# Tom-Ryder/VIforSDEs

Measured on AMD Instinct MI355X. Metric: sampled-paths/sec + ELBO-iters/sec (value = global_batch * ELBO-iters/s), higher is better.
Workload: dtype f32 (GRU/ELBO kernels) + bf16-autocast encoder; 1 GPU; lv: state_dim=2, T=400 (dt=0.1), batch=512/GPU, enc 256x8x4 heads, GRU 64x2; global_batch=512, parallelism=dp1, hip_graph=True

## Files before the change

### viforsdes_amd/csrc/vsde_common.h

```cpp
#pragma once
#include <hip/hip_runtime.h>
#include <stdint.h>
#include <stdio.h>
#include <stdlib.h>

#include "../../include/vsde_hip.h"

namespace vsde {

constexpr int kWave = 64;
constexpr int kHP = 64;
constexpr int kChunks = 16;
constexpr int kMatF4 = kChunks * 3 * kHP;

void set_error(const char *fmt, ...);

#ifdef VSDE_ABLATIONS
static inline long long vsde_knob(const char *name, long long dflt) {
    const char *e = getenv(name);
    return (e && *e) ? atoll(e) : dflt;
}
static inline int ablation_env(const char *name) {
    const char *e = getenv(name);
    const int v = e ? atoi(e) : 0;
// ... 22 lines not shown
        }                                                                            \
    } while (0)

struct RowView {
    const void *base;
    int64_t batch_stride;
    int64_t row_stride;
    int rows_per_batch;
    int shift;
    int col_split;
    int col_skip;
    int dtype;
};

__device__ __forceinline__ float bf16_to_f32(uint16_t v) { return __uint_as_float(((uint32_t)v) << 16); }

__device__ __forceinline__ int64_t rowview_offset(const RowView &v, int m, bool &valid) {
    int b = m / v.rows_per_batch;
    int t = m - b * v.rows_per_batch + v.shift;
    valid = t >= 0;
    return (int64_t)b * v.batch_stride + (int64_t)t * v.row_stride;
}

__device__ __forceinline__ float rowview_load(const RowView &v, int64_t off, int k) {
    int kk = k < v.col_split ? k : k + v.col_skip;
    if (v.dtype == 0) return ((const float *)v.base)[off + kk];
    return bf16_to_f32(((const uint16_t *)v.base)[off + kk]);
}

__device__ __forceinline__ float fast_rcp(float x) { return __builtin_amdgcn_rcpf(x); }
// ... 121 lines not shown
```

### viforsdes_amd/csrc/vsde_encoder.hip

```cpp
#include <stdlib.h>

#include "vsde_common.h"

namespace vsde {

struct bf16_t { uint16_t v; };

__device__ __forceinline__ float to_f32(float x) { return x; }
__device__ __forceinline__ float to_f32(bf16_t x) { return __uint_as_float(((uint32_t)x.v) << 16); }
template <typename T> __device__ __forceinline__ T from_f32(float x);
template <> __device__ __forceinline__ float from_f32<float>(float x) { return x; }
template <> __device__ __forceinline__ bf16_t from_f32<bf16_t>(float x) {
    uint32_t u = __float_as_uint(x);
    if ((u & 0x7fffffffu) > 0x7f800000u) return bf16_t{(uint16_t)((u >> 16) | 0x40)};
    u += 0x7fffu + ((u >> 16) & 1u);
    return bf16_t{(uint16_t)(u >> 16)};
}
template <typename T> __device__ __forceinline__ float rnd(float x) { return to_f32(from_f32<T>(x)); }

__device__ __forceinline__ float sigm(float x) { return fast_rcp(1.0f + __expf(-x)); }

template <typename T, int V> struct Pack;
template <int V> struct Pack<float, V> {
    static __device__ __forceinline__ void load(const float *p, float (&o)[V]) {
        if (V == 4) { float4 t = *(const float4 *)p; o[0] = t.x; o[1] = t.y; o[2] = t.z; o[3] = t.w; }
        else if (V == 2) { float2 t = *(const float2 *)p; o[0] = t.x; o[1] = t.y; }
        else {
#pragma unroll
            for (int i = 0; i < V; ++i) o[i] = p[i];
        }
    }
    static __device__ __forceinline__ void store(float *p, const float (&o)[V]) {
        if (V == 4) *(float4 *)p = make_float4(o[0], o[1], o[2], o[3]);
        else if (V == 2) *(float2 *)p = make_float2(o[0], o[1]);
        else {
#pragma unroll
            for (int i = 0; i < V; ++i) p[i] = o[i];
        }
    }
};
template <int V> struct Pack<bf16_t, V> {
    static __device__ __forceinline__ void load(const bf16_t *p, float (&o)[V]) {
        if (V == 8) { uint4 t = *(const uint4 *)p; const uint32_t w[4] = {t.x, t.y, t.z, t.w};
#pragma unroll
            for (int i = 0; i < 4; ++i) { o[2 * i] = __uint_as_float(w[i] << 16); o[2 * i + 1] = __uint_as_float(w[i] & 0xffff0000u); } }
        else if (V == 4) { uint2 t = *(const uint2 *)p; const uint32_t w[2] = {t.x, t.y};
#pragma unroll
            for (int i = 0; i < 2; ++i) { o[2 * i] = __uint_as_float(w[i] << 16); o[2 * i + 1] = __uint_as_float(w[i] & 0xffff0000u); } }
        else if (V == 2) { uint32_t w = *(const uint32_t *)p; o[0] = __uint_as_float(w << 16); o[1] = __uint_as_float(w & 0xffff0000u); }
        else {
#pragma unroll
            for (int i = 0; i < V; ++i) o[i] = to_f32(p[i]);
        }
    }
    static __device__ __forceinline__ void store(bf16_t *p, const float (&o)[V]) {
        if (V == 8 || V == 4 || V == 2) {
            uint32_t w[V / 2 > 0 ? V / 2 : 1];
#pragma unroll
            for (int i = 0; i < V / 2; ++i) w[i] = (uint32_t)from_f32<bf16_t>(o[2 * i]).v | ((uint32_t)from_f32<bf16_t>(o[2 * i + 1]).v << 16);
            if (V == 8) *(uint4 *)p = make_uint4(w[0], w[1], w[2 % (V / 2)], w[3 % (V / 2)]);
            else if (V == 4) *(uint2 *)p = make_uint2(w[0], w[1 % (V / 2)]);
            else *(uint32_t *)p = w[0];
        } else {
#pragma unroll
            for (int i = 0; i < V; ++i) p[i] = from_f32<bf16_t>(o[i]);
        }
    }
};
template <typename T> struct VecOf { static constexpr int v = 4; };
template <> struct VecOf<bf16_t> { static constexpr int v = 8; };

__device__ __forceinline__ float seg_sum(float v, int width) {
    for (int off = width >> 1; off > 0; off >>= 1) v += __shfl_xor(v, off, 64);
    return v;
}

template <typename T, int V, int LPR, int NSLAB>
__global__ void __launch_bounds__(256) ln_mod_fwd_kernel(const T *__restrict__ x, const T *__restrict__ scale,
                                                         const T *__restrict__ shift, T *__restrict__ y,
                                                         float *__restrict__ mean, float *__restrict__ rstd, int64_t M,
                                                         int N, int C, float eps, const T *__restrict__ res_y,
                                                         const T *__restrict__ res_gate, T *__restrict__ xnew, int64_t mp) {
    const int lane = threadIdx.x & (LPR - 1);
    constexpr int nslab = NSLAB;
    const int64_t stride = (int64_t)gridDim.x * (256 / LPR);
    int64_t m = (int64_t)blockIdx.x * (256 / LPR) + threadIdx.x / LPR;
    float v[NSLAB][V], ry[NSLAB][V], nv[NSLAB][V], nry[NSLAB][V];
    auto fetch = [&](int64_t mm, float (&vx)[NSLAB][V], float (&vy)[NSLAB][V]) {
#pragma unroll
        for (int sl = 0; sl < NSLAB; ++sl)
            if (sl < nslab) {
                Pack<T, V>::load(x + mm * C + (sl * LPR + lane) * V, vx[sl]);
                if (res_y) Pack<T, V>::load(res_y + mm * C + (sl * LPR + lane) * V, vy[sl]);
            }
    };
    if (m < M) fetch(m, v, ry);
    for (; m < M; m += stride) {
        const int64_t mn = m + stride;
        if (mn < M) fetch(mn, nv, nry);
        const int64_t b = m / N;
        float s = 0.f;
#pragma unroll
        for (int sl = 0; sl < NSLAB; ++sl)
            if (sl < nslab) {
                if (res_y) {
                    float rg[V];
                    Pack<T, V>::load(res_gate + b * mp + (sl * LPR + lane) * V, rg);
#pragma unroll
                    for (int e = 0; e < V; ++e) v[sl][e] = rnd<T>(v[sl][e] + rnd<T>(rg[e] * ry[sl][e]));
                    Pack<T, V>::store(xnew + m * C + (sl * LPR + lane) * V, v[sl]);
                }
#pragma unroll
                for (int e = 0; e < V; ++e) s += v[sl][e];
            }
        const float mu = seg_sum(s, LPR) / C;
        float q = 0.f;
#pragma unroll
        for (int sl = 0; sl < NSLAB; ++sl)
            if (sl < nslab)
#pragma unroll
                for (int e = 0; e < V; ++e) { const float d = v[sl][e] - mu; q += d * d; }
        const float rs = rsqrtf(seg_sum(q, LPR) / C + eps);
        if (lane == 0) { mean[m] = mu; rstd[m] = rs; }
#pragma unroll
        for (int sl = 0; sl < NSLAB; ++sl)
            if (sl < nslab) {
                const int c = (sl * LPR + lane) * V;
                float sc[V], sh[V], o[V];
                Pack<T, V>::load(scale + b * mp + c, sc); Pack<T, V>::load(shift + b * mp + c, sh);
#pragma unroll
                for (int e = 0; e < V; ++e) o[e] = (v[sl][e] - mu) * rs * (1.0f + sc[e]) + sh[e];
                Pack<T, V>::store(y + m * C + c, o);
            }
#pragma unroll
        for (int sl = 0; sl < NSLAB; ++sl)
#pragma unroll
            for (int e = 0; e < V; ++e) { v[sl][e] = nv[sl][e]; ry[sl][e] = nry[sl][e]; }
    }
}

constexpr int kColsumChunksMax = 64;
static int colsum_chunks(int64_t B, int N) {
    static int force = -1;
    if (force < 0) force = (int)vsde_knob("VSDE_COLSUM_CHUNKS", 0);
    if (force > 0) return force > kColsumChunksMax ? kColsumChunksMax : (force > N ? (N > 0 ? N : 1) : force);
    int64_t c = (768 + B - 1) / B;
    if (c < 4) c = 4;
    if (c > kColsumChunksMax) c = kColsumChunksMax;
    if (c > N / 8) c = N / 8 > 0 ? N / 8 : 1;
    return (int)c;
}

template <int NACC>
__device__ __forceinline__ void colsum_block_reduce(float *red, const float (&acc)[NACC], int slot, int slots, int lane_off,
                                                    int width, float *__restrict__ part, int C) {
    __syncthreads();
#pragma unroll
    for (int e = 0; e < NACC; ++e) red[slot * width + lane_off + e] = acc[e];
    __syncthreads();
    for (int c = threadIdx.x; c < width && c < C; c += blockDim.x) {
        float t = 0.f;
        for (int sidx = 0; sidx < slots; ++sidx) t += red[sidx * width + c];
        part[c] = t;
    }
}

template <typename T, int V, int LPR, int NSLAB>
__global__ void __launch_bounds__(256) ln_mod_bwd_kernel(const T *__restrict__ x, const T *__restrict__ scale,
                                                         const T *__restrict__ dy, const float *__restrict__ mean,
                                                         const float *__restrict__ rstd, const T *__restrict__ dres,
                                                         T *__restrict__ dx, float *__restrict__ part, int N, int C,
                                                         const T *__restrict__ res_y, const T *__restrict__ res_gate,
                                                         T *__restrict__ res_dy, int64_t mp) {
    extern __shared__ float red[];
    constexpr int SLOTS = 256 / LPR;
    const int lane = threadIdx.x & (LPR - 1), slot = threadIdx.x / LPR;
    const int b = blockIdx.y, nchunk = gridDim.x, B = gridDim.y;
    const int CL = (N + nchunk - 1) / nchunk;
    const int n0 = blockIdx.x * CL, n1 = min(N, n0 + CL);
    constexpr int nslab = NSLAB;
    float sc1[NSLAB][V], a1[NSLAB][V], a2[NSLAB][V], a3[NSLAB][V], gt[NSLAB][V];
#pragma unroll
    for (int sl = 0; sl < NSLAB; ++sl) {
        if (sl < nslab) {
            Pack<T, V>::load(scale + (int64_t)b * mp + (sl * LPR + lane) * V, sc1[sl]);
#pragma unroll
            for (int e = 0; e < V; ++e) sc1[sl][e] += 1.0f;
            if (res_y) Pack<T, V>::load(res_gate + (int64_t)b * mp + (sl * LPR + lane) * V, gt[sl]);
        }
#pragma unroll
        for (int e = 0; e < V; ++e) { a1[sl][e] = 0.f; a2[sl][e] = 0.f; a3[sl][e] = 0.f; }
    }
    for (int n = n0 + slot; n < n1; n += SLOTS) {
        const int64_t m = (int64_t)b * N + n;
        const float mu = mean[m], rs = rstd[m];
        float g[NSLAB][V], xh[NSLAB][V];
        float s1 = 0.f, s2 = 0.f;
#pragma unroll
        for (int sl = 0; sl < NSLAB; ++sl)
            if (sl < nslab) {
                const int c = (sl * LPR + lane) * V;
                Pack<T, V>::load(x + m * C + c, xh[sl]); Pack<T, V>::load(dy + m * C + c, g[sl]);
#pragma unroll
                for (int e = 0; e < V; ++e) {
                    xh[sl][e] = (xh[sl][e] - mu) * rs;
                    a1[sl][e] += g[sl][e] * xh[sl][e]; a2[sl][e] += g[sl][e];
                    g[sl][e] *= sc1[sl][e];
                    s1 += g[sl][e]; s2 += g[sl][e] * xh[sl][e];
                }
            }
        s1 = seg_sum(s1, LPR) / C; s2 = seg_sum(s2, LPR) / C;
#pragma unroll
        for (int sl = 0; sl < NSLAB; ++sl)
            if (sl < nslab) {
                const int c = (sl * LPR + lane) * V;
                float o[V];
#pragma unroll
                for (int e = 0; e < V; ++e) o[e] = rs * (g[sl][e] - s1 - xh[sl][e] * s2);
                if (dres) {
                    float r[V];
                    Pack<T, V>::load(dres + m * C + c, r);
#pragma unroll
                    for (int e = 0; e < V; ++e) o[e] += r[e];
                }
                Pack<T, V>::store(dx + m * C + c, o);
                if (res_y) {
                    float ry[V], od[V];
                    Pack<T, V>::load(res_y + m * C + c, ry);
#pragma unroll
                    for (int e = 0; e < V; ++e) { const float t = rnd<T>(o[e]); a3[sl][e] += t * ry[e]; od[e] = gt[sl][e] * t; }
                    Pack<T, V>::store(res_dy + m * C + c, od);
                }
            }
    }
    float *p0 = part + (((int64_t)0 * B + b) * nchunk + blockIdx.x) * C;
    float *p1 = part + (((int64_t)1 * B + b) * nchunk + blockIdx.x) * C;
#pragma unroll
    for (int sl = 0; sl < NSLAB; ++sl)
        if (sl < nslab) {
            const int off = sl * LPR * V;
            colsum_block_reduce<V>(red, a1[sl], slot, SLOTS, lane * V, LPR * V, p0 + off, C - off);
            colsum_block_reduce<V>(red, a2[sl], slot, SLOTS, lane * V, LPR * V, p1 + off, C - off);
            if (res_y) {
                float *p2 = part + (((int64_t)2 * B + b) * nchunk + blockIdx.x) * C;
                colsum_block_reduce<V>(red, a3[sl], slot, SLOTS, lane * V, LPR * V, p2 + off, C - off);
            }
        }
}

template <typename T, int V>
__global__ void __launch_bounds__(256) gated_residual_bwd_kernel(const T *__restrict__ y, const T *__restrict__ gate,
                                                                 const T *__restrict__ dout, T *__restrict__ dy,
                                                                 float *__restrict__ part, int N, int C, int64_t mp) {
    extern __shared__ float red[];
    const int lpt = C / V;
    const int slots = 256 / lpt;
    const int slot = threadIdx.x / lpt, lane = threadIdx.x - slot * lpt;
    const int b = blockIdx.y, nchunk = gridDim.x;
    const int CL = (N + nchunk - 1) / nchunk;
    const int n0 = blockIdx.x * CL, n1 = min(N, n0 + CL);
    const bool live = slot < slots;
    float gv[V], acc[V];
// ... 48 lines not shown
}

template <typename T, int V>
__global__ void __launch_bounds__(256) gated_residual_kernel(const T *__restrict__ x, const T *__restrict__ y,
                                                             const T *__restrict__ gate, T *__restrict__ out, int64_t total,
                                                             int N, int C, int mode, int64_t mp) {
    const int64_t stride = (int64_t)gridDim.x * blockDim.x * V;
    for (int64_t i0 = ((int64_t)blockIdx.x * blockDim.x + threadIdx.x) * V; i0 < total; i0 += stride) {
        const int64_t m = i0 / C;
        const int c = (int)(i0 - m * C);
        const int64_t b = m / N;
        float gv[V], yv[V], xv[V], o[V];
        Pack<T, V>::load(gate + b * mp + c, gv); Pack<T, V>::load(y + i0, yv);
        if (mode == 0) Pack<T, V>::load(x + i0, xv);
#pragma unroll
        for (int e = 0; e < V; ++e) { const float g = gv[e] * yv[e]; o[e] = mode == 0 ? xv[e] + rnd<T>(g) : g; }
        Pack<T, V>::store(out + i0, o);
    }
}

template <typename T, int V>
__global__ void __launch_bounds__(256) swiglu_fwd_kernel(const T *__restrict__ u, T *__restrict__ out, int64_t M, int H2) {
    const int hv = H2 / V;
    const int64_t total = M * hv, stride = (int64_t)gridDim.x * blockDim.x;
    for (int64_t i = (int64_t)blockIdx.x * blockDim.x + threadIdx.x; i < total; i += stride) {
        const int64_t m = i / hv;
        const int j = (int)(i - m * hv) * V;
        float a[V], bv[V], o[V];
        Pack<T, V>::load(u + m * 2 * H2 + j, a); Pack<T, V>::load(u + m * 2 * H2 + H2 + j, bv);
#pragma unroll
        for (int e = 0; e < V; ++e) o[e] = rnd<T>(a[e] * sigm(a[e])) * bv[e];
        Pack<T, V>::store(out + m * H2 + j, o);
    }
}

template <typename T, int V>
__global__ void __launch_bounds__(256) swiglu_bwd_kernel(const T *__restrict__ u, const T *__restrict__ dout, T *__restrict__ du,
                                                         int64_t M, int H2) {
    const int hv = H2 / V;
    const int64_t total = M * hv, stride = (int64_t)gridDim.x * blockDim.x;
    for (int64_t i = (int64_t)blockIdx.x * blockDim.x + threadIdx.x; i < total; i += stride) {
        const int64_t m = i / hv;
        const int j = (int)(i - m * hv) * V;
        float a[V], bv[V], g[V], da[V], db[V];
        Pack<T, V>::load(u + m * 2 * H2 + j, a); Pack<T, V>::load(u + m * 2 * H2 + H2 + j, bv); Pack<T, V>::load(dout + m * H2 + j, g);
#pragma unroll
// ... 7 lines not shown

template <typename T, int V>
__global__ void __launch_bounds__(256) gate_merge_fwd_kernel(const T *__restrict__ attn, const T *__restrict__ glog,
                                                             T *__restrict__ out, int64_t M, int N, int heads, int d, int token_major,
                                                             int64_t gstride) {
    const int C = heads * d, cv = C / V;
    const int64_t total = M * cv, stride = (int64_t)gridDim.x * blockDim.x;
    for (int64_t i = (int64_t)blockIdx.x * blockDim.x + threadIdx.x; i < total; i += stride) {
        const int64_t m = i / cv;
        const int c = (int)(i - m * cv) * V, hh = c / d, k = c - hh * d;
        const int64_t b = m / N, n = m - b * N;
        float gl[V], av[V], o[V];
        Pack<T, V>::load(glog + m * gstride + k, gl);
        Pack<T, V>::load(attn + (token_major ? m * C + c : ((b * heads + hh) * N + n) * d + k), av);
#pragma unroll
        for (int e = 0; e < V; ++e) o[e] = av[e] * rnd<T>(sigm(gl[e]));
        Pack<T, V>::store(out + m * C + c, o);
    }
}

template <typename T, int V>
__global__ void __launch_bounds__(256) gate_merge_bwd_kernel(const T *__restrict__ attn, const T *__restrict__ glog,
                                                             const T *__restrict__ dout, T *__restrict__ dattn,
                                                             T *__restrict__ dglog, int64_t M, int N, int heads, int d, int token_major,
                                                             int64_t gstride) {
    const int C = heads * d, dv = d / V;
    const int64_t total = M * dv, stride = (int64_t)gridDim.x * blockDim.x;
    for (int64_t i = (int64_t)blockIdx.x * blockDim.x + threadIdx.x; i < total; i += stride) {
        const int64_t m = i / dv;
        const int k = (int)(i - m * dv) * V;
        const int64_t b = m / N, n = m - b * N;
// ... 37 lines not shown
    if (ok) {
#pragma unroll
        for (int t = 0; t < 3; ++t) { Pack<T, PV>::load(row + t * C + i, x[2 * t]); Pack<T, PV>::load(row + t * C + i + half, x[2 * t + 1]); }
    }
    float sq = 0.f, sk = 0.f;
#pragma unroll
    for (int e = 0; e < PV; ++e) { sq += x[0][e] * x[0][e] + x[1][e] * x[1][e]; sk += x[2][e] * x[2][e] + x[3][e] * x[3][e]; }
    const float rq = rsqrtf(seg_sum(sq, tph) / d + eps);
    const float rk = rsqrtf(seg_sum(sk, tph) / d + eps);
    if (!ok) return;
    float cs[PV], sn[PV], wql[PV], wqh[PV], wkl[PV], wkh[PV];
    Pack<float, PV>::load(cosT + n * half + i, cs); Pack<float, PV>::load(sinT + n * half + i, sn);
    Pack<float, PV>::load(wq + i, wql); Pack<float, PV>::load(wq + i + half, wqh);
    Pack<float, PV>::load(wk + i, wkl); Pack<float, PV>::load(wk + i + half, wkh);
    const int64_t o = token_major ? (m * heads + hh) * d + i : ((b * heads + hh) * N + n) * d + i;
    float o0[PV], o1[PV];
#pragma unroll
    for (int e = 0; e < PV; ++e) {
        const float a0 = rnd<T>(x[0][e] * rq * wql[e]), a1 = rnd<T>(x[1][e] * rq * wqh[e]);
        o0[e] = a0 * cs[e] - a1 * sn[e]; o1[e] = a0 * sn[e] + a1 * cs[e];
    }
    Pack<T, PV>::store(q + o, o0); Pack<T, PV>::store(q + o + half, o1);
#pragma unroll
    for (int e = 0; e < PV; ++e) {
        const float a0 = rnd<T>(x[2][e] * rk * wkl[e]), a1 = rnd<T>(x[3][e] * rk * wkh[e]);
        o0[e] = a0 * cs[e] - a1 * sn[e]; o1[e] = a0 * sn[e] + a1 * cs[e];
    }
    Pack<T, PV>::store(k + o, o0); Pack<T, PV>::store(k + o + half, o1);
    if (v0) {
        const float l = lam[0];
        float p0[PV], p1[PV];
        Pack<T, PV>::load(v0 + o, p0); Pack<T, PV>::load(v0 + o + half, p1);
#pragma unroll
        for (int e = 0; e < PV; ++e) { x[4][e] = l * x[4][e] + (1.0f - l) * p0[e]; x[5][e] = l * x[5][e] + (1.0f - l) * p1[e]; }
    }
    Pack<T, PV>::store(v + o, x[4]); Pack<T, PV>::store(v + o + half, x[5]);
}

template <typename T, int PV>
__global__ void __launch_bounds__(256) qk_norm_rope_bwd_kernel(const T *__restrict__ qkv, const float *__restrict__ cosT,
                                                               const float *__restrict__ sinT, const float *__restrict__ wq,
                                                               const float *__restrict__ wk, const T *__restrict__ v0,
// ... 23 lines not shown
        float cs[PV], sn[PV], g0[PV], g1[PV];
        Pack<float, PV>::load(cosT + n * half + i, cs); Pack<float, PV>::load(sinT + n * half + i, sn);
#pragma unroll
        for (int t = 0; t < 2; ++t) {
            Pack<T, PV>::load(row + t * C + i, x[2 * t]); Pack<T, PV>::load(row + t * C + i + half, x[2 * t + 1]);
            Pack<T, PV>::load((t == 0 ? dq : dk) + o, g0); Pack<T, PV>::load((t == 0 ? dq : dk) + o + half, g1);
            Pack<float, PV>::load((t == 0 ? wq : wk) + i, w[2 * t]); Pack<float, PV>::load((t == 0 ? wq : wk) + i + half, w[2 * t + 1]);
#pragma unroll
            for (int e = 0; e < PV; ++e) { gy[2 * t][e] = g0[e] * cs[e] + g1[e] * sn[e]; gy[2 * t + 1][e] = -g0[e] * sn[e] + g1[e] * cs[e]; }
        }
        Pack<T, PV>::load(dv + o, g0); Pack<T, PV>::load(dv + o + half, g1);
        if (dv_extra) {
            float e0[PV], e1[PV];
            Pack<T, PV>::load(dv_extra + o, e0); Pack<T, PV>::load(dv_extra + o + half, e1);
#pragma unroll
            for (int e = 0; e < PV; ++e) { g0[e] = rnd<T>(g0[e] + e0[e]); g1[e] = rnd<T>(g1[e] + e1[e]); }
        }
        if (v0) {
            const float l = lam[0];
            float a0[PV], a1[PV], p0[PV], p1[PV], z0[PV], z1[PV];
            Pack<T, PV>::load(row + 2 * C + i, a0); Pack<T, PV>::load(row + 2 * C + i + half, a1);
            Pack<T, PV>::load(v0 + o, p0); Pack<T, PV>::load(v0 + o + half, p1);
#pragma unroll
            for (int e = 0; e < PV; ++e) {
                dlam += g0[e] * (a0[e] - p0[e]) + g1[e] * (a1[e] - p1[e]);
                z0[e] = (1.0f - l) * g0[e]; z1[e] = (1.0f - l) * g1[e]; g0[e] *= l; g1[e] *= l;
            }
            if (dv0_accumulate) {
                float y0[PV], y1[PV];
                Pack<T, PV>::load(dv0 + o, y0); Pack<T, PV>::load(dv0 + o + half, y1);
#pragma unroll
                for (int e = 0; e < PV; ++e) { z0[e] = y0[e] + rnd<T>(z0[e]); z1[e] = y1[e] + rnd<T>(z1[e]); }
            }
            Pack<T, PV>::store(dv0 + o, z0); Pack<T, PV>::store(dv0 + o + half, z1);
        }
        Pack<T, PV>::store(drow + 2 * C + i, g0); Pack<T, PV>::store(drow + 2 * C + i + half, g1);
    }
#pragma unroll
    for (int t = 0; t < 2; ++t) {
        float ss = 0.f, dt = 0.f;
#pragma unroll
        for (int e = 0; e < PV; ++e) {
            ss += x[2 * t][e] * x[2 * t][e] + x[2 * t + 1][e] * x[2 * t + 1][e];
            dt += x[2 * t][e] * w[2 * t][e] * gy[2 * t][e] + x[2 * t + 1][e] * w[2 * t + 1][e] * gy[2 * t + 1][e];
        }
        const float r = rsqrtf(seg_sum(ss, tph) / d + eps);
        const float dot = seg_sum(dt, tph) / d;
// ... 35 lines not shown

template <typename T>
static int ln_mod_dispatch(int which, const void *x, const void *scale, const void *shift_or_dy, const void *dres, void *out,
                           float *mean, float *rstd, float *part, int64_t B, int N, int C, float eps, hipStream_t s,
                           LnResidual res = LnResidual()) {
    VSDE_CHECK_ARG(C % 64 == 0 && C <= 1024, VSDE_E_BADARG, "ln_modulate needs C %% 64 == 0 and C <= 1024, got %d", C);
    constexpr int VF = VecOf<T>::v;
    const int64_t M = B * N;
    dim3 block(256);
#define LNM_N(V, LPR, NS)                                                                                                     \
    do {                                                                                                                      \
        if (which == 0) {                                                                                                     \
            int64_t nblk = (M + 256 / LPR - 1) / (256 / LPR);                                                                 \
            const int64_t cap = ln_fwd_grid_cap();                                                                            \
            dim3 grid((unsigned)(nblk < cap ? nblk : cap));                                                                   \
            hipLaunchKernelGGL((ln_mod_fwd_kernel<T, V, LPR, NS>), grid, block, 0, s, (const T *)x, (const T *)scale,         \
                               (const T *)shift_or_dy, (T *)out, mean, rstd, M, N, C, eps, (const T *)res.y,                  \
                               (const T *)res.gate, (T *)res.out, res.mp ? res.mp : (int64_t)C);                              \
        } else {                                                                                                              \
            hipLaunchKernelGGL((ln_mod_bwd_kernel<T, V, LPR, NS>), dim3(colsum_chunks(B, N), (unsigned)B), block,                   \
                               256 * V * sizeof(float), s, (const T *)x, (const T *)scale, (const T *)shift_or_dy,            \
                               (const float *)mean, (const float *)rstd, (const T *)dres, (T *)out, part, N, C,               \
                               (const T *)res.y, (const T *)res.gate, (T *)res.out, res.mp ? res.mp : (int64_t)C);            \
        }                                                                                                                     \
    } while (0)
#define LNM(V, LPR)                                                                                                           \
    do {                                                                                                                      \
        switch (C / ((LPR) * (V))) {                                                                                          \
            case 1: LNM_N(V, LPR, 1); break;                                                                                  \
            case 2: LNM_N(V, LPR, 2); break;                                                                                  \
            case 3: LNM_N(V, LPR, 3); break;                                                                                  \
            default: LNM_N(V, LPR, 4); break;                                                                                 \
        }                                                                                                                     \
// ... 261 lines not shown
```

### viforsdes_amd/csrc/vsde_linear.hip

```cpp
#include <stdlib.h>

#include "vsde_common.h"

namespace vsde {

typedef float f32x16 __attribute__((ext_vector_type(16)));
typedef short bf16x8 __attribute__((ext_vector_type(8)));
typedef uint32_t u32x4 __attribute__((ext_vector_type(4)));

constexpr int EPI_PLAIN = 0, EPI_SWIGLU = 1, EPI_SWIGLU_BWD = 2, EPI_QKNORM = 3, EPI_GATE_BWD = 4;
constexpr int R2_THREADS = 256, R2_SLD = 88;

struct LinParams {
    const uint16_t *A; int64_t lda;
    const uint16_t *W;
    const uint16_t *bias;
    uint16_t *C; int64_t ldc;
    uint16_t *S; int64_t lds_;
    const uint16_t *U; int64_t ldu;
    int64_t M; int N, K;
    int chunks;
    int tail_local, tail_chunks;
    uint16_t *Qo, *Ko, *Vo, *Go; int64_t ldg;
    const float *cosT, *sinT, *wq, *wk, *lam;
    const uint16_t *V0;
    int heads, tokens; float eps;
    int gate_sigmoid;
    const uint16_t *Og; const uint16_t *Sg; int64_t ldsg;
    uint16_t *Dgate; int64_t lddg;
    float *Delta;
    float *Rinv;
    uint16_t *Vdiff;
    const uint16_t *Gate; int64_t ldgate;
    int dbg;
    int xstage;
};

typedef __bf16 hwbf16x2 __attribute__((ext_vector_type(2)));
typedef float f32x2 __attribute__((ext_vector_type(2)));
__device__ __forceinline__ uint32_t pack_bf16x2(float lo, float hi) {
    const f32x2 v = {lo, hi};
    return __builtin_bit_cast(uint32_t, __builtin_convertvector(v, hwbf16x2));
}
__device__ __forceinline__ float bf_lo(uint32_t w) { return __uint_as_float(w << 16); }
__device__ __forceinline__ float bf_hi(uint32_t w) { return __uint_as_float(w & 0xffff0000u); }
__device__ __forceinline__ float rbf(float x) { return (float)(__bf16)x; }
__device__ __forceinline__ void lds_barrier() { asm volatile("s_waitcnt lgkmcnt(0)\n\ts_barrier" ::: "memory"); }

__device__ __forceinline__ float sigm_f(float x) { return fast_rcp(1.0f + __expf(-x)); }

template <int SLD, int R>
__device__ __forceinline__ void flush_rows64(const uint16_t *stage, uint16_t *dst, int64_t ld, int64_t row0, int64_t M, int lane) {
#pragma unroll
    for (int i = 0; i < R / 8; ++i) {
        const int row = (lane >> 3) + 8 * i, c = lane & 7;
        const u32x4 v = *(const u32x4 *)(stage + row * SLD + c * 8);
        if (row0 + row < M) __builtin_nontemporal_store(v, (u32x4 *)(dst + (row0 + row) * ld + c * 8));
    }
// ... 936 lines not shown
```

Before: 19930 paths/s.

## Prefetch LayerNorm-modulation rows as raw bf16 and use hardware bf16 conversion

Rewrites the encoder's modulated LayerNorm forward and backward kernels. Raw packed bf16 words for x, residual, gate, scale and shift are now double-buffered, so the next row's loads are issued before the current row is processed. The residual and dres branches are specialised at compile time, and the per-row batch index is tracked incrementally instead of dividing. Segment reductions use swizzle, DPP and permlane ops, and software round-to-nearest bf16 conversion is replaced by the hardware packed convert. More registers are held live, which could lower occupancy, and NaN handling in the conversion may differ slightly.

```diff
diff --git a/viforsdes_amd/csrc/vsde_common.h b/viforsdes_amd/csrc/vsde_common.h
--- a/viforsdes_amd/csrc/vsde_common.h
+++ b/viforsdes_amd/csrc/vsde_common.h
@@ -60,6 +60,14 @@
 };
 
 __device__ __forceinline__ float bf16_to_f32(uint16_t v) { return __uint_as_float(((uint32_t)v) << 16); }
+
+typedef __bf16 hwbf16x2_t __attribute__((ext_vector_type(2)));
+typedef float f32x2_t __attribute__((ext_vector_type(2)));
+__device__ __forceinline__ uint32_t pack_bf16x2(float lo, float hi) {
+    const f32x2_t v = {lo, hi};
+    return __builtin_bit_cast(uint32_t, __builtin_convertvector(v, hwbf16x2_t));
+}
+__device__ __forceinline__ uint16_t f32_to_bf16(float x) { return __builtin_bit_cast(uint16_t, (__bf16)x); }
 
 __device__ __forceinline__ int64_t rowview_offset(const RowView &v, int m, bool &valid) {
     int b = m / v.rows_per_batch;
diff --git a/viforsdes_amd/csrc/vsde_encoder.hip b/viforsdes_amd/csrc/vsde_encoder.hip
--- a/viforsdes_amd/csrc/vsde_encoder.hip
+++ b/viforsdes_amd/csrc/vsde_encoder.hip
@@ -10,18 +10,19 @@
 __device__ __forceinline__ float to_f32(bf16_t x) { return __uint_as_float(((uint32_t)x.v) << 16); }
 template <typename T> __device__ __forceinline__ T from_f32(float x);
 template <> __device__ __forceinline__ float from_f32<float>(float x) { return x; }
-template <> __device__ __forceinline__ bf16_t from_f32<bf16_t>(float x) {
-    uint32_t u = __float_as_uint(x);
-    if ((u & 0x7fffffffu) > 0x7f800000u) return bf16_t{(uint16_t)((u >> 16) | 0x40)};
-    u += 0x7fffu + ((u >> 16) & 1u);
-    return bf16_t{(uint16_t)(u >> 16)};
-}
+template <> __device__ __forceinline__ bf16_t from_f32<bf16_t>(float x) { return bf16_t{f32_to_bf16(x)}; }
 template <typename T> __device__ __forceinline__ float rnd(float x) { return to_f32(from_f32<T>(x)); }
+
+__device__ __forceinline__ float add_unfused(float a, float b) {
+#pragma clang fp contract(off)
+    return a + b;
+}
 
 __device__ __forceinline__ float sigm(float x) { return fast_rcp(1.0f + __expf(-x)); }
 
 template <typename T, int V> struct Pack;
 template <int V> struct Pack<float, V> {
+    struct Raw { float f[V]; };
     static __device__ __forceinline__ void load(const float *p, float (&o)[V]) {
         if (V == 4) { float4 t = *(const float4 *)p; o[0] = t.x; o[1] = t.y; o[2] = t.z; o[3] = t.w; }
         else if (V == 2) { float2 t = *(const float2 *)p; o[0] = t.x; o[1] = t.y; }
@@ -38,34 +39,48 @@
             for (int i = 0; i < V; ++i) p[i] = o[i];
         }
     }
+    static __device__ __forceinline__ Raw load_raw(const float *p) { Raw r; load(p, r.f); return r; }
+    static __device__ __forceinline__ void unpack(const Raw &r, float (&o)[V]) {
+#pragma unroll
+        for (int i = 0; i < V; ++i) o[i] = r.f[i];
+    }
+    static __device__ __forceinline__ void round(float (&)[V]) {}
+    static __device__ __forceinline__ void round_store(float *p, float (&o)[V]) { store(p, o); }
 };
 template <int V> struct Pack<bf16_t, V> {
-    static __device__ __forceinline__ void load(const bf16_t *p, float (&o)[V]) {
-        if (V == 8) { uint4 t = *(const uint4 *)p; const uint32_t w[4] = {t.x, t.y, t.z, t.w};
-#pragma unroll
-            for (int i = 0; i < 4; ++i) { o[2 * i] = __uint_as_float(w[i] << 16); o[2 * i + 1] = __uint_as_float(w[i] & 0xffff0000u); } }
-        else if (V == 4) { uint2 t = *(const uint2 *)p; const uint32_t w[2] = {t.x, t.y};
-#pragma unroll
-            for (int i = 0; i < 2; ++i) { o[2 * i] = __uint_as_float(w[i] << 16); o[2 * i + 1] = __uint_as_float(w[i] & 0xffff0000u); } }
-        else if (V == 2) { uint32_t w = *(const uint32_t *)p; o[0] = __uint_as_float(w << 16); o[1] = __uint_as_float(w & 0xffff0000u); }
-        else {
-#pragma unroll
-            for (int i = 0; i < V; ++i) o[i] = to_f32(p[i]);
-        }
-    }
-    static __device__ __forceinline__ void store(bf16_t *p, const float (&o)[V]) {
-        if (V == 8 || V == 4 || V == 2) {
-            uint32_t w[V / 2 > 0 ? V / 2 : 1];
-#pragma unroll
-            for (int i = 0; i < V / 2; ++i) w[i] = (uint32_t)from_f32<bf16_t>(o[2 * i]).v | ((uint32_t)from_f32<bf16_t>(o[2 * i + 1]).v << 16);
-            if (V == 8) *(uint4 *)p = make_uint4(w[0], w[1], w[2 % (V / 2)], w[3 % (V / 2)]);
-            else if (V == 4) *(uint2 *)p = make_uint2(w[0], w[1 % (V / 2)]);
-            else *(uint32_t *)p = w[0];
-        } else {
-#pragma unroll
-            for (int i = 0; i < V; ++i) p[i] = from_f32<bf16_t>(o[i]);
-        }
-    }
+    static_assert(V == 8 || V == 4 || V == 2 || V == 1, "bf16 rows move as 16, 8, 4 or 2 bytes per lane");
+    static constexpr int NW = V > 1 ? V / 2 : 1;
+    struct Raw { uint32_t w[NW]; };
+    static __device__ __forceinline__ Raw load_raw(const bf16_t *p) {
+        Raw r;
+        if (V == 8) { uint4 t = *(const uint4 *)p; r.w[0] = t.x; r.w[1 % NW] = t.y; r.w[2 % NW] = t.z; r.w[3 % NW] = t.w; }
+        else if (V == 4) { uint2 t = *(const uint2 *)p; r.w[0] = t.x; r.w[1 % NW] = t.y; }
+        else if (V == 2) r.w[0] = *(const uint32_t *)p;
+        else r.w[0] = p[0].v;
+        return r;
+    }
+    static __device__ __forceinline__ void unpack(const Raw &r, float (&o)[V]) {
+        if (V == 1) { o[0] = __uint_as_float(r.w[0] << 16); return; }
+#pragma unroll
+        for (int i = 0; i < V / 2; ++i) { o[(2 * i) % V] = __uint_as_float(r.w[i] << 16); o[(2 * i + 1) % V] = __uint_as_float(r.w[i] & 0xffff0000u); }
+    }
+    static __device__ __forceinline__ Raw pack(const float (&o)[V]) {
+        Raw r;
+        if (V == 1) { r.w[0] = f32_to_bf16(o[0]); return r; }
+#pragma unroll
+        for (int i = 0; i < V / 2; ++i) r.w[i] = pack_bf16x2(o[(2 * i) % V], o[(2 * i + 1) % V]);
+        return r;
+    }
+    static __device__ __forceinline__ void store_raw(bf16_t *p, const Raw &r) {
+        if (V == 8) *(uint4 *)p = make_uint4(r.w[0], r.w[1 % NW], r.w[2 % NW], r.w[3 % NW]);
+        else if (V == 4) *(uint2 *)p = make_uint2(r.w[0], r.w[1 % NW]);
+        else if (V == 2) *(uint32_t *)p = r.w[0];
+        else p[0].v = (uint16_t)r.w[0];
+    }
+    static __device__ __forceinline__ void load(const bf16_t *p, float (&o)[V]) { unpack(load_raw(p), o); }
+    static __device__ __forceinline__ void store(bf16_t *p, const float (&o)[V]) { store_raw(p, pack(o)); }
+    static __device__ __forceinline__ void round(float (&o)[V]) { unpack(pack(o), o); }
+    static __device__ __forceinline__ void round_store(bf16_t *p, float (&o)[V]) { const Raw r = pack(o); store_raw(p, r); unpack(r, o); }
 };
 template <typename T> struct VecOf { static constexpr int v = 4; };
 template <> struct VecOf<bf16_t> { static constexpr int v = 8; };
@@ -73,6 +88,101 @@
 __device__ __forceinline__ float seg_sum(float v, int width) {
     for (int off = width >> 1; off > 0; off >>= 1) v += __shfl_xor(v, off, 64);
     return v;
+}
+
+template <int W> __device__ __forceinline__ void seg_sum2(float &a, float &b) {
+    static_assert(W == 64 || W == 32, "a token is 32 or 64 lanes");
+    if (W > 32) { a = sum_xor32(a); b = sum_xor32(b); }
+    { const float ta = xor_lane<16>(a), tb = xor_lane<16>(b); a += ta; b += tb; }
+    { const float ta = xor_lane<8>(a), tb = xor_lane<8>(b); a += ta; b += tb; }
+    { const float ta = xor_lane<4>(a), tb = xor_lane<4>(b); a += ta; b += tb; }
+    a = dpp_add<0x4e>(a); b = dpp_add<0x4e>(b);
+    a = dpp_add<0xb1>(a); b = dpp_add<0xb1>(b);
+}
+template <int W> __device__ __forceinline__ float seg_sum1(float a) {
+    static_assert(W == 64 || W == 32, "a token is 32 or 64 lanes");
+    if (W > 32) a = sum_xor32(a);
+    a += xor_lane<16>(a); a += xor_lane<8>(a); a += xor_lane<4>(a);
+    return dpp_add<0xb1>(dpp_add<0x4e>(a));
+}
+
+template <typename T, int V, int NSLAB> struct LnFwdSet { typename Pack<T, V>::Raw x[NSLAB], y[NSLAB], g[NSLAB], sc[NSLAB], sh[NSLAB]; };
+
+template <typename T, int V, int LPR, int NSLAB, bool RES>
+__device__ __forceinline__ void ln_mod_fwd_body(const T *__restrict__ x, const T *__restrict__ scale, const T *__restrict__ shift,
+                                                T *__restrict__ y, float *__restrict__ mean, float *__restrict__ rstd, int64_t M,
+                                                int N, int C, float eps, const T *__restrict__ res_y,
+                                                const T *__restrict__ res_gate, T *__restrict__ xnew, int64_t mp, int stride_b,
+                                                int stride_n) {
+    typedef Pack<T, V> P;
+    typedef LnFwdSet<T, V, NSLAB> Set;
+    constexpr int SLOTS = 256 / LPR;
+    const int lane = threadIdx.x & (LPR - 1);
+    const int64_t stride = (int64_t)gridDim.x * SLOTS;
+    int64_t m = (int64_t)blockIdx.x * SLOTS + threadIdx.x / LPR;
+    if (m >= M) return;
+    const int64_t b0 = m / N;
+    int n = (int)(m - b0 * N);
+    int64_t orow = m * C + lane * V;
+    int64_t omod = b0 * mp + lane * V;
+    const int64_t drow = stride * C, dmod = (int64_t)stride_b * mp;
+    auto fetch = [&](int64_t o, int64_t om, Set &f) {
+#pragma unroll
+        for (int sl = 0; sl < NSLAB; ++sl) {
+            f.x[sl] = P::load_raw(x + o + sl * LPR * V);
+            if (RES) { f.y[sl] = P::load_raw(res_y + o + sl * LPR * V); f.g[sl] = P::load_raw(res_gate + om + sl * LPR * V); }
+            f.sc[sl] = P::load_raw(scale + om + sl * LPR * V); f.sh[sl] = P::load_raw(shift + om + sl * LPR * V);
+        }
+    };
+    auto trip = [&](const Set &cur, Set &nxt, const int ahead) {
+        const bool more = ahead == 1 || m + stride < M;
+        int nn = n + stride_n;
+        int64_t omn = omod + dmod;
+        if (nn >= N) { nn -= N; omn += mp; }
+        const int64_t orn = more ? orow + drow : orow;
+        omn = more ? omn : omod;
+        if (ahead) fetch(orn, omn, nxt);
+        __builtin_amdgcn_sched_barrier(0);
+        float v[NSLAB][V];
+        float s = 0.f;
+#pragma unroll
+        for (int sl = 0; sl < NSLAB; ++sl) {
+            P::unpack(cur.x[sl], v[sl]);
+            if (RES) {
+                float ry[V], rg[V];
+                P::unpack(cur.y[sl], ry); P::unpack(cur.g[sl], rg);
+#pragma unroll
+                for (int e = 0; e < V; ++e) ry[e] = rg[e] * ry[e];
+                P::round(ry);
+#pragma unroll
+                for (int e = 0; e < V; ++e) v[sl][e] = v[sl][e] + ry[e];
+                P::round_store(xnew + orow + sl * LPR * V, v[sl]);
+            }
+#pragma unroll
+            for (int e = 0; e < V; ++e) s += v[sl][e];
+        }
+        const float mu = seg_sum1<LPR>(s) / C;
+        float q = 0.f;
+#pragma unroll
+        for (int sl = 0; sl < NSLAB; ++sl)
+#pragma unroll
+            for (int e = 0; e < V; ++e) { const float d = v[sl][e] - mu; q += d * d; }
+        const float rs = rsqrtf(seg_sum1<LPR>(q) / C + eps);
+        if (lane == 0) { mean[m] = mu; rstd[m] = rs; }
+#pragma unroll
+        for (int sl = 0; sl < NSLAB; ++sl) {
+            float sc[V], sh[V], o[V];
+            P::unpack(cur.sc[sl], sc); P::unpack(cur.sh[sl], sh);
+#pragma unroll
+            for (int e = 0; e < V; ++e) o[e] = (v[sl][e] - mu) * rs * (1.0f + sc[e]) + sh[e];
+            P::store(y + orow + sl * LPR * V, o);
+        }
+        m += stride; n = nn; orow = orn; omod = omn;
+    };
+    Set sa, sb;
+    fetch(orow, omod, sa);
+    while (m + stride < M) { trip(sa, sb, 1); trip(sb, sa, 2); }
+    if (m < M) trip(sa, sb, 0);
 }
 
 template <typename T, int V, int LPR, int NSLAB>
@@ -80,63 +190,10 @@
                                                          const T *__restrict__ shift, T *__restrict__ y,
                                                          float *__restrict__ mean, float *__restrict__ rstd, int64_t M,
                                                          int N, int C, float eps, const T *__restrict__ res_y,
-                                                         const T *__restrict__ res_gate, T *__restrict__ xnew, int64_t mp) {
-    const int lane = threadIdx.x & (LPR - 1);
-    constexpr int nslab = NSLAB;
-    const int64_t stride = (int64_t)gridDim.x * (256 / LPR);
-    int64_t m = (int64_t)blockIdx.x * (256 / LPR) + threadIdx.x / LPR;
-    float v[NSLAB][V], ry[NSLAB][V], nv[NSLAB][V], nry[NSLAB][V];
-    auto fetch = [&](int64_t mm, float (&vx)[NSLAB][V], float (&vy)[NSLAB][V]) {
-#pragma unroll
-        for (int sl = 0; sl < NSLAB; ++sl)
-            if (sl < nslab) {
-                Pack<T, V>::load(x + mm * C + (sl * LPR + lane) * V, vx[sl]);
-                if (res_y) Pack<T, V>::load(res_y + mm * C + (sl * LPR + lane) * V, vy[sl]);
-            }
-    };
-    if (m < M) fetch(m, v, ry);
-    for (; m < M; m += stride) {
-        const int64_t mn = m + stride;
-        if (mn < M) fetch(mn, nv, nry);
-        const int64_t b = m / N;
-        float s = 0.f;
-#pragma unroll
-        for (int sl = 0; sl < NSLAB; ++sl)
-            if (sl < nslab) {
-                if (res_y) {
-                    float rg[V];
-                    Pack<T, V>::load(res_gate + b * mp + (sl * LPR + lane) * V, rg);
-#pragma unroll
-                    for (int e = 0; e < V; ++e) v[sl][e] = rnd<T>(v[sl][e] + rnd<T>(rg[e] * ry[sl][e]));
-                    Pack<T, V>::store(xnew + m * C + (sl * LPR + lane) * V, v[sl]);
-                }
-#pragma unroll
-                for (int e = 0; e < V; ++e) s += v[sl][e];
-            }
-        const float mu = seg_sum(s, LPR) / C;
-        float q = 0.f;
-#pragma unroll
-        for (int sl = 0; sl < NSLAB; ++sl)
-            if (sl < nslab)
-#pragma unroll
-                for (int e = 0; e < V; ++e) { const float d = v[sl][e] - mu; q += d * d; }
-        const float rs = rsqrtf(seg_sum(q, LPR) / C + eps);
-        if (lane == 0) { mean[m] = mu; rstd[m] = rs; }
-#pragma unroll
-        for (int sl = 0; sl < NSLAB; ++sl)
-            if (sl < nslab) {
-                const int c = (sl * LPR + lane) * V;
-                float sc[V], sh[V], o[V];
-                Pack<T, V>::load(scale + b * mp + c, sc); Pack<T, V>::load(shift + b * mp + c, sh);
-#pragma unroll
-                for (int e = 0; e < V; ++e) o[e] = (v[sl][e] - mu) * rs * (1.0f + sc[e]) + sh[e];
-                Pack<T, V>::store(y + m * C + c, o);
-            }
-#pragma unroll
-        for (int sl = 0; sl < NSLAB; ++sl)
-#pragma unroll
-            for (int e = 0; e < V; ++e) { v[sl][e] = nv[sl][e]; ry[sl][e] = nry[sl][e]; }
-    }
+                                                         const T *__restrict__ res_gate, T *__restrict__ xnew, int64_t mp,
+                                                         int stride_b, int stride_n) {
+    if (res_y) ln_mod_fwd_body<T, V, LPR, NSLAB, true>(x, scale, shift, y, mean, rstd, M, N, C, eps, res_y, res_gate, xnew, mp, stride_b, stride_n);
+    else ln_mod_fwd_body<T, V, LPR, NSLAB, false>(x, scale, shift, y, mean, rstd, M, N, C, eps, res_y, res_gate, xnew, mp, stride_b, stride_n);
 }
 
 constexpr int kColsumChunksMax = 64;
@@ -165,6 +222,114 @@
     }
 }
 
+template <typename T, int V, int NSLAB> struct LnBwdSet { typename Pack<T, V>::Raw x[NSLAB], g[NSLAB], r[NSLAB], y[NSLAB]; float mu, rs; };
+
+template <typename T, int V, int LPR, int NSLAB, bool DRES, bool RES>
+__device__ __forceinline__ void ln_mod_bwd_body(float *red, const T *__restrict__ x, const T *__restrict__ scale,
+                                                const T *__restrict__ dy, const float *__restrict__ mean,
+                                                const float *__restrict__ rstd, const T *__restrict__ dres, T *__restrict__ dx,
+                                                float *__restrict__ part, int N, int C, const T *__restrict__ res_y,
+                                                const T *__restrict__ res_gate, T *__restrict__ res_dy, int64_t mp) {
+    typedef Pack<T, V> P;
+    typedef LnBwdSet<T, V, NSLAB> Set;
+    constexpr int SLOTS = 256 / LPR;
+    const int lane = threadIdx.x & (LPR - 1), slot = threadIdx.x / LPR;
+    const int b = blockIdx.y, nchunk = gridDim.x, B = gridDim.y;
+    const int CL = (N + nchunk - 1) / nchunk;
+    const int n0 = blockIdx.x * CL, n1 = min(N, n0 + CL);
+    float sc1[NSLAB][V], a1[NSLAB][V], a2[NSLAB][V], a3[NSLAB][V];
+    typename P::Raw gt[NSLAB];
+#pragma unroll
+    for (int sl = 0; sl < NSLAB; ++sl) {
+        P::load(scale + (int64_t)b * mp + (sl * LPR + lane) * V, sc1[sl]);
+#pragma unroll
+        for (int e = 0; e < V; ++e) sc1[sl][e] += 1.0f;
+        if (RES) gt[sl] = P::load_raw(res_gate + (int64_t)b * mp + (sl * LPR + lane) * V);
+#pragma unroll
+        for (int e = 0; e < V; ++e) { a1[sl][e] = 0.f; a2[sl][e] = 0.f; a3[sl][e] = 0.f; }
+    }
+    int n = n0 + slot;
+    if (n < n1) {
+        int64_t m = (int64_t)b * N + n;
+        int64_t orow = m * C + lane * V;
+        const int64_t drow = (int64_t)SLOTS * C;
+        auto fetch = [&](int64_t mm, int64_t o, Set &f) {
+            f.mu = mean[mm]; f.rs = rstd[mm];
+#pragma unroll
+            for (int sl = 0; sl < NSLAB; ++sl) {
+                f.x[sl] = P::load_raw(x + o + sl * LPR * V); f.g[sl] = P::load_raw(dy + o + sl * LPR * V);
+                if (DRES) f.r[sl] = P::load_raw(dres + o + sl * LPR * V);
+                if (RES) f.y[sl] = P::load_raw(res_y + o + sl * LPR * V);
+            }
+        };
+        auto trip = [&](const Set &cur, Set &nxt, const int ahead) {
+            const bool more = ahead == 1 || n + SLOTS < n1;
+            const int64_t mn = more ? m + SLOTS : m, orn = more ? orow + drow : orow;
+            if (ahead) fetch(mn, orn, nxt);
+            __builtin_amdgcn_sched_barrier(0);
+            const float mu = cur.mu, rs = cur.rs;
+            float g[NSLAB][V], xh[NSLAB][V];
+            float s1 = 0.f, s2 = 0.f;
+#pragma unroll
+            for (int sl = 0; sl < NSLAB; ++sl) {
+                P::unpack(cur.x[sl], xh[sl]); P::unpack(cur.g[sl], g[sl]);
+#pragma unroll
+                for (int e = 0; e < V; ++e) {
+                    xh[sl][e] = (xh[sl][e] - mu) * rs;
+                    a1[sl][e] += g[sl][e] * xh[sl][e]; a2[sl][e] += g[sl][e];
+                    g[sl][e] *= sc1[sl][e];
+                    s1 += g[sl][e]; s2 += g[sl][e] * xh[sl][e];
+                }
+            }
+            seg_sum2<LPR>(s1, s2);
+            s1 = s1 / C; s2 = s2 / C;
+#pragma unroll
+            for (int sl = 0; sl < NSLAB; ++sl) {
+                float o[V];
+#pragma unroll
+                for (int e = 0; e < V; ++e) o[e] = rs * (g[sl][e] - s1 - xh[sl][e] * s2);
+                if (DRES) {
+                    float r[V];
+                    P::unpack(cur.r[sl], r);
+#pragma unroll
+                    for (int e = 0; e < V; ++e) o[e] = add_unfused(o[e], r[e]);
+                }
+                if (RES) {
+                    float ry[V], gv[V], od[V];
+                    P::round_store(dx + orow + sl * LPR * V, o);
+                    P::unpack(cur.y[sl], ry); P::unpack(gt[sl], gv);
+#pragma unroll
+                    for (int e = 0; e < V; ++e) { a3[sl][e] += o[e] * ry[e]; od[e] = gv[e] * o[e]; }
+                    P::store(res_dy + orow + sl * LPR * V, od);
+                } else {
+                    P::store(dx + orow + sl * LPR * V, o);
+                }
+            }
+            n += SLOTS; m = mn; orow = orn;
+        };
+        Set sa, sb;
+        if (NSLAB * V * sizeof(T) <= 16) {
+            fetch(m, orow, sa);
+            while (n + SLOTS < n1) { trip(sa, sb, 1); trip(sb, sa, 2); }
+            if (n < n1) trip(sa, sb, 0);
+        } else {
+            for (; n < n1;) { fetch(m, orow, sa); trip(sa, sb, 0); }
+        }
+    }
+    float *p0 = part + (((int64_t)0 * B + b) * nchunk + blockIdx.x) * C;
+    float *p1 = part + (((int64_t)1 * B + b) * nchunk + blockIdx.x) * C;
+#pragma unroll
+    for (int sl = 0; sl < NSLAB; ++sl) {
+        const int off = sl * LPR * V;
+        colsum_block_reduce<V>(red, a1[sl], slot, SLOTS, lane * V, LPR * V, p0 + off, C - off);
+        colsum_block_reduce<V>(red, a2[sl], slot, SLOTS, lane * V, LPR * V, p1 + off, C - off);
+        if (RES) {
+            float *p2 = part + (((int64_t)2 * B + b) * nchunk + blockIdx.x) * C;
+            colsum_block_reduce<V>(red, a3[sl], slot, SLOTS, lane * V, LPR * V, p2 + off, C - off);
+        }
+    }
+}
+
 template <typename T, int V, int LPR, int NSLAB>
 __global__ void __launch_bounds__(256) ln_mod_bwd_kernel(const T *__restrict__ x, const T *__restrict__ scale,
                                                          const T *__restrict__ dy, const float *__restrict__ mean,
@@ -173,79 +338,10 @@
                                                          const T *__restrict__ res_y, const T *__restrict__ res_gate,
                                                          T *__restrict__ res_dy, int64_t mp) {
     extern __shared__ float red[];
-    constexpr int SLOTS = 256 / LPR;
-    const int lane = threadIdx.x & (LPR - 1), slot = threadIdx.x / LPR;
-    const int b = blockIdx.y, nchunk = gridDim.x, B = gridDim.y;
-    const int CL = (N + nchunk - 1) / nchunk;
-    const int n0 = blockIdx.x * CL, n1 = min(N, n0 + CL);
-    constexpr int nslab = NSLAB;
-    float sc1[NSLAB][V], a1[NSLAB][V], a2[NSLAB][V], a3[NSLAB][V], gt[NSLAB][V];
-#pragma unroll
-    for (int sl = 0; sl < NSLAB; ++sl) {
-        if (sl < nslab) {
-            Pack<T, V>::load(scale + (int64_t)b * mp + (sl * LPR + lane) * V, sc1[sl]);
-#pragma unroll
-            for (int e = 0; e < V; ++e) sc1[sl][e] += 1.0f;
-            if (res_y) Pack<T, V>::load(res_gate + (int64_t)b * mp + (sl * LPR + lane) * V, gt[sl]);
-        }
-#pragma unroll
-        for (int e = 0; e < V; ++e) { a1[sl][e] = 0.f; a2[sl][e] = 0.f; a3[sl][e] = 0.f; }
-    }
-    for (int n = n0 + slot; n < n1; n += SLOTS) {
-        const int64_t m = (int64_t)b * N + n;
-        const float mu = mean[m], rs = rstd[m];
-        float g[NSLAB][V], xh[NSLAB][V];
-        float s1 = 0.f, s2 = 0.f;
-#pragma unroll
-        for (int sl = 0; sl < NSLAB; ++sl)
-            if (sl < nslab) {
-                const int c = (sl * LPR + lane) * V;
-                Pack<T, V>::load(x + m * C + c, xh[sl]); Pack<T, V>::load(dy + m * C + c, g[sl]);
-#pragma unroll
-                for (int e = 0; e < V; ++e) {
-                    xh[sl][e] = (xh[sl][e] - mu) * rs;
-                    a1[sl][e] += g[sl][e] * xh[sl][e]; a2[sl][e] += g[sl][e];
-                    g[sl][e] *= sc1[sl][e];
-                    s1 += g[sl][e]; s2 += g[sl][e] * xh[sl][e];
-                }
-            }
-        s1 = seg_sum(s1, LPR) / C; s2 = seg_sum(s2, LPR) / C;
-#pragma unroll
-        for (int sl = 0; sl < NSLAB; ++sl)
-            if (sl < nslab) {
-                const int c = (sl * LPR + lane) * V;
-                float o[V];
-#pragma unroll
-                for (int e = 0; e < V; ++e) o[e] = rs * (g[sl][e] - s1 - xh[sl][e] * s2);
-                if (dres) {
-                    float r[V];
-                    Pack<T, V>::load(dres + m * C + c, r);
-#pragma unroll
-                    for (int e = 0; e < V; ++e) o[e] += r[e];
-                }
-                Pack<T, V>::store(dx + m * C + c, o);
-                if (res_y) {
-                    float ry[V], od[V];
-                    Pack<T, V>::load(res_y + m * C + c, ry);
-#pragma unroll
-                    for (int e = 0; e < V; ++e) { const float t = rnd<T>(o[e]); a3[sl][e] += t * ry[e]; od[e] = gt[sl][e] * t; }
-                    Pack<T, V>::store(res_dy + m * C + c, od);
-                }
-            }
-    }
-    float *p0 = part + (((int64_t)0 * B + b) * nchunk + blockIdx.x) * C;
-    float *p1 = part + (((int64_t)1 * B + b) * nchunk + blockIdx.x) * C;
-#pragma unroll
-    for (int sl = 0; sl < NSLAB; ++sl)
-        if (sl < nslab) {
-            const int off = sl * LPR * V;
-            colsum_block_reduce<V>(red, a1[sl], slot, SLOTS, lane * V, LPR * V, p0 + off, C - off);
-            colsum_block_reduce<V>(red, a2[sl], slot, SLOTS, lane * V, LPR * V, p1 + off, C - off);
-            if (res_y) {
-                float *p2 = part + (((int64_t)2 * B + b) * nchunk + blockIdx.x) * C;
-                colsum_block_reduce<V>(red, a3[sl], slot, SLOTS, lane * V, LPR * V, p2 + off, C - off);
-            }
-        }
+#define LN_BWD_BODY(DRES, RES) ln_mod_bwd_body<T, V, LPR, NSLAB, DRES, RES>(red, x, scale, dy, mean, rstd, dres, dx, part, N, C, res_y, res_gate, res_dy, mp)
+    if (res_y) { if (dres) LN_BWD_BODY(true, true); else LN_BWD_BODY(false, true); }
+    else { if (dres) LN_BWD_BODY(true, false); else LN_BWD_BODY(false, false); }
+#undef LN_BWD_BODY
 }
 
 template <typename T, int V>
@@ -324,7 +420,12 @@
         Pack<T, V>::load(gate + b * mp + c, gv); Pack<T, V>::load(y + i0, yv);
         if (mode == 0) Pack<T, V>::load(x + i0, xv);
 #pragma unroll
-        for (int e = 0; e < V; ++e) { const float g = gv[e] * yv[e]; o[e] = mode == 0 ? xv[e] + rnd<T>(g) : g; }
+        for (int e = 0; e < V; ++e) o[e] = gv[e] * yv[e];
+        if (mode == 0) {
+            Pack<T, V>::round(o);
+#pragma unroll
+            for (int e = 0; e < V; ++e) o[e] = xv[e] + o[e];
+        }
         Pack<T, V>::store(out + i0, o);
     }
 }
@@ -339,7 +440,10 @@
         float a[V], bv[V], o[V];
         Pack<T, V>::load(u + m * 2 * H2 + j, a); Pack<T, V>::load(u + m * 2 * H2 + H2 + j, bv);
 #pragma unroll
-        for (int e = 0; e < V; ++e) o[e] = rnd<T>(a[e] * sigm(a[e])) * bv[e];
+        for (int e = 0; e < V; ++e) o[e] = a[e] * sigm(a[e]);
+        Pack<T, V>::round(o);
+#pragma unroll
+        for (int e = 0; e < V; ++e) o[e] = o[e] * bv[e];
         Pack<T, V>::store(out + m * H2 + j, o);
     }
 }
@@ -377,7 +481,10 @@
         Pack<T, V>::load(glog + m * gstride + k, gl);
         Pack<T, V>::load(attn + (token_major ? m * C + c : ((b * heads + hh) * N + n) * d + k), av);
 #pragma unroll
-        for (int e = 0; e < V; ++e) o[e] = av[e] * rnd<T>(sigm(gl[e]));
+        for (int e = 0; e < V; ++e) gl[e] = sigm(gl[e]);
+        Pack<T, V>::round(gl);
+#pragma unroll
+        for (int e = 0; e < V; ++e) o[e] = av[e] * gl[e];
         Pack<T, V>::store(out + m * C + c, o);
     }
 }
@@ -445,18 +552,18 @@
     Pack<float, PV>::load(wq + i, wql); Pack<float, PV>::load(wq + i + half, wqh);
     Pack<float, PV>::load(wk + i, wkl); Pack<float, PV>::load(wk + i + half, wkh);
     const int64_t o = token_major ? (m * heads + hh) * d + i : ((b * heads + hh) * N + n) * d + i;
-    float o0[PV], o1[PV];
-#pragma unroll
-    for (int e = 0; e < PV; ++e) {
-        const float a0 = rnd<T>(x[0][e] * rq * wql[e]), a1 = rnd<T>(x[1][e] * rq * wqh[e]);
-        o0[e] = a0 * cs[e] - a1 * sn[e]; o1[e] = a0 * sn[e] + a1 * cs[e];
-    }
+    float o0[PV], o1[PV], a0[PV], a1[PV];
+#pragma unroll
+    for (int e = 0; e < PV; ++e) { a0[e] = x[0][e] * rq * wql[e]; a1[e] = x[1][e] * rq * wqh[e]; }
+    Pack<T, PV>::round(a0); Pack<T, PV>::round(a1);
+#pragma unroll
+    for (int e = 0; e < PV; ++e) { o0[e] = a0[e] * cs[e] - a1[e] * sn[e]; o1[e] = a0[e] * sn[e] + a1[e] * cs[e]; }
     Pack<T, PV>::store(q + o, o0); Pack<T, PV>::store(q + o + half, o1);
 #pragma unroll
-    for (int e = 0; e < PV; ++e) {
-        const float a0 = rnd<T>(x[2][e] * rk * wkl[e]), a1 = rnd<T>(x[3][e] * rk * wkh[e]);
-        o0[e] = a0 * cs[e] - a1 * sn[e]; o1[e] = a0 * sn[e] + a1 * cs[e];
-    }
+    for (int e = 0; e < PV; ++e) { a0[e] = x[2][e] * rk * wkl[e]; a1[e] = x[3][e] * rk * wkh[e]; }
+    Pack<T, PV>::round(a0); Pack<T, PV>::round(a1);
+#pragma unroll
+    for (int e = 0; e < PV; ++e) { o0[e] = a0[e] * cs[e] - a1[e] * sn[e]; o1[e] = a0[e] * sn[e] + a1[e] * cs[e]; }
     Pack<T, PV>::store(k + o, o0); Pack<T, PV>::store(k + o + half, o1);
     if (v0) {
         const float l = lam[0];
@@ -510,7 +617,8 @@
             float e0[PV], e1[PV];
             Pack<T, PV>::load(dv_extra + o, e0); Pack<T, PV>::load(dv_extra + o + half, e1);
 #pragma unroll
-            for (int e = 0; e < PV; ++e) { g0[e] = rnd<T>(g0[e] + e0[e]); g1[e] = rnd<T>(g1[e] + e1[e]); }
+            for (int e = 0; e < PV; ++e) { g0[e] = g0[e] + e0[e]; g1[e] = g1[e] + e1[e]; }
+            Pack<T, PV>::round(g0); Pack<T, PV>::round(g1);
         }
         if (v0) {
             const float l = lam[0];
@@ -525,8 +633,9 @@
             if (dv0_accumulate) {
                 float y0[PV], y1[PV];
                 Pack<T, PV>::load(dv0 + o, y0); Pack<T, PV>::load(dv0 + o + half, y1);
-#pragma unroll
-                for (int e = 0; e < PV; ++e) { z0[e] = y0[e] + rnd<T>(z0[e]); z1[e] = y1[e] + rnd<T>(z1[e]); }
+                Pack<T, PV>::round(z0); Pack<T, PV>::round(z1);
+#pragma unroll
+                for (int e = 0; e < PV; ++e) { z0[e] = y0[e] + z0[e]; z1[e] = y1[e] + z1[e]; }
             }
             Pack<T, PV>::store(dv0 + o, z0); Pack<T, PV>::store(dv0 + o + half, z1);
         }
@@ -592,9 +701,11 @@
             int64_t nblk = (M + 256 / LPR - 1) / (256 / LPR);                                                                 \
             const int64_t cap = ln_fwd_grid_cap();                                                                            \
             dim3 grid((unsigned)(nblk < cap ? nblk : cap));                                                                   \
+            const int64_t stride = (int64_t)grid.x * (256 / LPR);                       \
             hipLaunchKernelGGL((ln_mod_fwd_kernel<T, V, LPR, NS>), grid, block, 0, s, (const T *)x, (const T *)scale,         \
                                (const T *)shift_or_dy, (T *)out, mean, rstd, M, N, C, eps, (const T *)res.y,                  \
-                               (const T *)res.gate, (T *)res.out, res.mp ? res.mp : (int64_t)C);                              \
+                               (const T *)res.gate, (T *)res.out, res.mp ? res.mp : (int64_t)C, (int)(stride / N),           \
+                               (int)(stride % N));                                                                            \
         } else {                                                                                                              \
             hipLaunchKernelGGL((ln_mod_bwd_kernel<T, V, LPR, NS>), dim3(colsum_chunks(B, N), (unsigned)B), block,                   \
                                256 * V * sizeof(float), s, (const T *)x, (const T *)scale, (const T *)shift_or_dy,            \
diff --git a/viforsdes_amd/csrc/vsde_linear.hip b/viforsdes_amd/csrc/vsde_linear.hip
--- a/viforsdes_amd/csrc/vsde_linear.hip
+++ b/viforsdes_amd/csrc/vsde_linear.hip
@@ -36,12 +36,6 @@
     int xstage;
 };
 
-typedef __bf16 hwbf16x2 __attribute__((ext_vector_type(2)));
-typedef float f32x2 __attribute__((ext_vector_type(2)));
-__device__ __forceinline__ uint32_t pack_bf16x2(float lo, float hi) {
-    const f32x2 v = {lo, hi};
-    return __builtin_bit_cast(uint32_t, __builtin_convertvector(v, hwbf16x2));
-}
 __device__ __forceinline__ float bf_lo(uint32_t w) { return __uint_as_float(w << 16); }
 __device__ __forceinline__ float bf_hi(uint32_t w) { return __uint_as_float(w & 0xffff0000u); }
 __device__ __forceinline__ float rbf(float x) { return (float)(__bf16)x; }
```

Measured after the change: 20200 paths/s, median of 6. +1.4%, better.
